# fizzy74/passport-zk-circuits

Measured on AMD Instinct MI355X. Metric: registerIdentityBuilder witnesses/sec, batch=4096, 1 & 8 MI355X; % HBM roofline, higher is better.
Workload: dtype bn254_fr (u32 limbs)

## Files before the change

### passport-zk-circuits_amd/csrc/host_api.cpp

```cpp
#include <string.h>

#include <algorithm>

#include "../../include/pzkwit.h"
#include "host_api.hpp"
#include "pos_prog.hpp"

namespace pzk {

int nsets_env(bool query) {
  const char* e = getenv("PZK_NSETS");
  const int v = e ? atoi(e) : query ? 6 : 3;
  return v < 2 ? 2 : v > PIPELINE_SETS_MAX ? PIPELINE_SETS_MAX : v;
}

bool parse_sym(const char* text, size_t len, uint64_t o0_size, std::vector<uint32_t>& inv, std::string& why) {
  std::vector<int64_t> w_of;
  size_t i = 0;
  uint64_t line = 0;
  auto num = [&](int64_t& v) -> bool {
    bool neg = false, any = false;
    v = 0;
    if (i < len && text[i] == '-') { neg = true; i++; }
    while (i < len && text[i] >= '0' && text[i] <= '9') { v = v * 10 + (text[i] - '0'); i++; any = true; if (v > (1ll << 40)) return false; }
    if (neg) v = -v;
    return any;
  };
  while (i < len) {
    line++;
    if (text[i] == '\n' || text[i] == '\r') { i++; continue; }
    int64_t sig, wit, comp;
    if (!num(sig) || i >= len || text[i++] != ',' || !num(wit) || i >= len || text[i++] != ',' || !num(comp)) {
      why = "sym line " + std::to_string(line) + ": expected signal_idx,witness_idx,component_idx,name";
      return false;
    }
    while (i < len && text[i] != '\n') i++;
    if (sig < 1 || (uint64_t)sig >= o0_size) {
      why = "sym line " + std::to_string(line) + ": signal index " + std::to_string(sig) + " outside 1.." +
            std::to_string(o0_size - 1);
      return false;
    }
    if (wit == -1) continue;
    if (wit < 1 || (uint64_t)wit >= o0_size) {
      why = "sym line " + std::to_string(line) + ": witness index " + std::to_string(wit) + " outside 1.." +
            std::to_string(o0_size - 1);
      return false;
    }
    if ((uint64_t)wit >= w_of.size()) w_of.resize(wit + 1, -1);
    if (w_of[wit] == -1 || sig < w_of[wit]) w_of[wit] = sig;
  }
  if (w_of.size() < 2) { why = "sym: no signal is kept"; return false; }
  inv.assign(w_of.size(), 0);
  for (size_t k = 1; k < w_of.size(); k++) {
    if (w_of[k] < 0) { why = "sym: witness index " + std::to_string(k) + " is not assigned"; return false; }
    inv[k] = (uint32_t)w_of[k];
  }
  return true;
}

void map_program(const Layout& lay, const std::vector<uint32_t>& inv, bool force_gather, MapProgram& out) {
  out = MapProgram();
  bool monotone = true;
  for (size_t k = 1; k < inv.size() && monotone; k++) monotone = inv[k] > inv[k - 1];
  if (!monotone || force_gather) return;
  out.direct = true;
  const size_t nw = lay.wit_size / 64 + 3;
  out.bits.assign(nw, 0);
  out.rank.assign(nw, 0);
  for (uint32_t g : inv) out.bits[g >> 6] |= 1ull << (g & 63);
  for (size_t i = 1; i < nw; i++) out.rank[i] = out.rank[i - 1] + (uint32_t)__builtin_popcountll(out.bits[i - 1]);
  auto kept = [&](uint64_t g) { return (out.bits[g >> 6] >> (g & 63)) & 1; };
  bool mix_t[POS_MAX_T + 1] = {};
  auto kept_in = [&](uint64_t a, uint64_t n) {
    uint64_t c = 0;
    for (uint64_t g = a; g < a + n; g++) c += kept(g);
    return c;
  };
  for (int e : {E_SHA, E_SHAD, E_POS, E_ECT}) {
    std::vector<Work>& wl = out.work[e];
    wl = lay.work[e];
    if (e == E_SHA || e == E_SHAD) {
      std::vector<Work> merged;
      uint64_t kept_cur = 0;
      for (const Work& wk : wl) {
        const uint64_t k = kept_in(lay.regions[wk.region].off + wk.start, wk.count);
        Work* last = merged.empty() ? nullptr : &merged.back();
        if (last && last->region == wk.region && lay.regions[wk.region].kind == RK_SHA_BLOCK &&
            last->start + last->count == wk.start && kept_cur + k <= EMIT_CHUNK) {
          last->count += wk.count;
          kept_cur += k;
        } else {
          merged.push_back(wk);
          kept_cur = k;
        }
      }
      wl.swap(merged);
    }
    for (Work& wk : wl) {
      const Region& R = lay.regions[wk.region];
      const uint32_t* src = nullptr;
      const uint16_t* src16 = nullptr;
      if (R.kind == RK_SHA_BLOCK) src = lay.sha_prog.data() + wk.start;
      else if (R.kind == RK_POSEIDON) src16 = lay.pos_prog.data() + lay.pos_prog_off[lay.pos[R.a[0]].n + 1] + wk.start;
      else if (R.kind == RK_ECT) src = lay.ec_prog.data() + lay.ec_prog_off[R.a[1]] + wk.start;
      else continue;
      wk.pad = (uint32_t)out.mprog.size();
      for (uint32_t q = 0; q < wk.count; q++)
        if (kept(R.off + wk.start + q)) {
          out.mprog.push_back(src ? src[q] : src16[q]);
          if (src16) mix_t[lay.pos[R.a[0]].n + 1] |= (pos_img_need_t(lay.pos[R.a[0]].n + 1, src16[q]) & PI_MIX) != 0;
        }
    }
  }
  for (int t = 2; t <= POS_MAX_T; t++)
    if (!mix_t[t]) out.pos_nomix |= 1u << t;
  if (out.mprog.empty()) out.mprog.push_back(0);
}

}

using namespace pzk;

extern "C" {

static int sym_check_impl(const pzk_params* params, const char* sym, size_t sym_len, uint64_t* witness_size) {
  if (!params || !sym) return api_fail(PZK_E_ARG, "null argument");
  Layout L;
  std::string why;
  if (!build_layout(*params, L, why)) return api_fail(PZK_E_PARAMS, why);
  std::vector<uint32_t> inv;
  if (!parse_sym(sym, sym_len, L.wit_size, inv, why)) return api_fail(PZK_E_ARG, why);
  if (witness_size) *witness_size = inv.size();
  return 0;
}

static int layout_query_impl(const pzk_params* params, pzk_info* info, uint32_t* n_regions) {
  if (!params || !info) return api_fail(PZK_E_ARG, "null argument");
  Layout L;
  std::string why;
  if (!build_layout(*params, L, why)) return api_fail(PZK_E_PARAMS, why);
  memset(info, 0, sizeof *info);
  info->witness_size = L.wit_size;
  info->n_inputs = L.n_inputs;
  info->n_outputs = L.n_outputs;
  info->n_public_inputs = L.n_public;
  info->n_input_groups = (uint32_t)L.inputs.size();
  info->pipeline_depth = nsets_env(params->circuit == PZK_CIRCUIT_QUERY);
  if (n_regions) *n_regions = (uint32_t)L.regions.size();
  return 0;
}

static int layout_region_impl(const pzk_params* params, uint32_t i, uint64_t* off, uint32_t* len, uint32_t* kind) {
  if (!params) return api_fail(PZK_E_ARG, "null argument");
  Layout L;
  std::string why;
  if (!build_layout(*params, L, why)) return api_fail(PZK_E_PARAMS, why);
  if (i >= L.regions.size()) return api_fail(PZK_E_ARG, "region index out of range");
  if (off) *off = L.regions[i].off;
  if (len) *len = L.regions[i].len;
  if (kind) *kind = L.regions[i].kind;
  return 0;
}

int pzk_sym_check(const pzk_params* params, const char* sym, size_t sym_len, uint64_t* witness_size) {
  return guarded([&] { return sym_check_impl(params, sym, sym_len, witness_size); });
}

int pzk_layout_query(const pzk_params* params, pzk_info* info, uint32_t* n_regions) {
  return guarded([&] { return layout_query_impl(params, info, n_regions); });
}

int pzk_layout_region(const pzk_params* params, uint32_t i, uint64_t* off, uint32_t* len, uint32_t* kind) {
  return guarded([&] { return layout_region_impl(params, i, off, len, kind); });
}

}
```

### passport-zk-circuits_amd/csrc/kernels.hip

```cpp
#include <hip/hip_runtime.h>
#include <stdlib.h>
#include <string.h>

#include "poseidon.hpp"
#include "regcore.hpp"
#include "smt_chain4.hpp"
#include "pss.hpp"
#include "regemit.hpp"
#include "sha.hpp"
#include "sha1.hpp"
#include "sha512.hpp"
#include "sha_prog.hpp"
#include "mapsink.hpp"
#include "kernels.hpp"

namespace pzk {

__global__ void k_load_values(const ValueLoad* loads, int n_loads, const uint8_t* inputs, uint64_t n_inputs,
                              fr* values, uint32_t batch) {
  uint32_t w = blockIdx.x * blockDim.x + threadIdx.x;
  int l = blockIdx.y;
  if (w >= batch || l >= n_loads) return;
  ValueLoad ld = loads[l];
  fr x = load_fr(inputs + 32ull * ((uint64_t)w * n_inputs + ld.in_off));
  values[(size_t)ld.slot * batch + w] = fr_to_mont(x);
}

__global__ void __launch_bounds__(64, 1) k_sha_core(const ShaJob* jobs, int n_jobs, const uint8_t* inputs, uint64_t n_inputs,
                           const uint8_t* derived, uint64_t n_derived, uint32_t* sha_core, uint32_t core_words,
                           int32_t* status, uint32_t batch) {
  core_priority();
  uint32_t w = blockIdx.x * blockDim.x + threadIdx.x;
  int j = blockIdx.y;
  if (w >= batch || j >= n_jobs) return;
  const ShaJob& J = jobs[j];
  const uint8_t* row = J.src ? derived + 32ull * (uint64_t)w * n_derived : inputs + 32ull * (uint64_t)w * n_inputs;
  if (J.algo == 1) sha1_core_lane(row, J, sha_core + (size_t)w * core_words, status ? status + w : nullptr);
  else if (J.algo >= 3) sha512_core_lane(row, J, sha_core + (size_t)w * core_words, status ? status + w : nullptr);
  else sha_core_lane(row, J, sha_core + (size_t)w * core_words, status ? status + w : nullptr);
}

__device__ __forceinline__ uint64_t sha_own_sig(const Region& R, const uint32_t* H , uint32_t s,
                                                bool& is_copy, uint64_t& src) {
  const int B = R.a[1];
  const uint32_t inLen = 512u * B, O = R.a[4] == 224 ? 224u : 256u;
  is_copy = false;
  if (R.a[3]) {
    if (s < O) { uint32_t j = s >> 5, i = s & 31; return (H[B * 8 + j] >> (31 - i)) & 1; }
    s -= O;
    if (s < inLen) { is_copy = true; src = (uint64_t)R.a[2] + s; return 0; }
    s -= inLen;
  }
  if (s < O) { uint32_t j = s >> 5, i = s & 31; return (H[B * 8 + j] >> (31 - i)) & 1; }
  s -= O;
  if (s < inLen) { is_copy = true; src = (uint64_t)R.a[2] + s; return 0; }
  s -= inLen;
  if (s < 256u * (B + 1)) { uint32_t m = s >> 8, j = (s >> 5) & 7, i = s & 31; return (H[m * 8 + j] >> i) & 1; }
  s -= 256u * (B + 1);
  return ((O == 224 ? SHA224_IV[s >> 5] : SHA_IV[s >> 5]) >> (s & 31)) & 1;
}

template <int SHA_U, int MM>
__global__ void __launch_bounds__(EMIT_THREADS) k_emit_sha(DevLayout L, const Work* work, const uint8_t* inputs,
                                                          const uint8_t* derived, const uint32_t* sha_core,
                                                          uint8_t* wtns, size_t stride, int wit_major) {
  __shared__ uint32_t core[SHA_BLOCK_CORE + 8 * 65];
  __shared__ __attribute__((aligned(16))) uint64_t wt[SHA_WT_SIZE];
  const Work wk = work[wit_major ? blockIdx.y : blockIdx.x];
  const uint32_t w = wit_major ? blockIdx.x : blockIdx.y;
  const Region R = L.regions[wk.region];
  const ShaJob job = L.sha[R.a[0]];
  const uint32_t* wc = sha_core + (size_t)w * L.sha_core_words + job.core_off;
  const OutRow out = out_row(L, wtns, stride, w, R.off + wk.start);
  if (R.kind == RK_SHA_BLOCK) {
    const uint32_t* bc = wc + R.a[1] * SHA_BLOCK_CORE;
    for (int i = threadIdx.x; i < SHA_BLOCK_CORE; i += blockDim.x) core[i] = bc[i];
    __syncthreads();
    const ShaBlk Bk{core};
    const uint32_t a = wk.start, b = wk.start + wk.count - 1;
    auto rng = [](uint32_t lo_sig, uint32_t per, int nr, uint32_t x) {
      return x < lo_sig ? 0 : (int)min((x - lo_sig) / per, (uint32_t)nr - 1);
    };
    const bool sch = a < SHA_SCH_ROUND0 + 48 * SHA_SCH_ROUND_SIGS && b >= SHA_SCH_ROUND0;
    const bool cmp = a < SHA_RDS_CMP0 + 64 * SHA_CMP_SIGS && b >= SHA_RDS_CMP0;
    const int r0 = sch ? rng(SHA_SCH_ROUND0, SHA_SCH_ROUND_SIGS, 48, a) : 0;
    const int r1 = sch ? rng(SHA_SCH_ROUND0, SHA_SCH_ROUND_SIGS, 48, b) + 1 : 0;
    const int k0 = cmp ? rng(SHA_RDS_CMP0, SHA_CMP_SIGS, 64, a) : 0;
    const int k1 = cmp ? rng(SHA_RDS_CMP0, SHA_CMP_SIGS, 64, b) + 1 : 0;
    const int n_base = SHA_WT_SCH, n_ff = 16, n_sch = (r1 - r0) * SHA_SCH_WORDS, n_cmp = (k1 - k0) * SHA_CMP_WORDS;
    for (int v = threadIdx.x; v < n_base + n_ff + n_sch + n_cmp; v += blockDim.x) {
      int e = v < n_base ? v
            : v < n_base + n_ff ? SHA_WT_FF32 + (v - n_base)
            : v < n_base + n_ff + n_sch ? SHA_WT_SCH + r0 * SHA_SCH_WORDS + (v - n_base - n_ff)
                                        : SHA_WT_CMP + k0 * SHA_CMP_WORDS + (v - n_base - n_ff - n_sch);
      wt[e] = sha_wt_entry(Bk, e);
    }
    __syncthreads();
    const DescRun dr = desc_run<MM>(L, wtns, stride, w, wk, R.off + wk.start, L.sha_prog + wk.start);
    const uint32_t* prog = dr.prog;
    const uint32_t tot = 2 * dr.count;
    for (uint32_t base = threadIdx.x; base < tot; base += SHA_U * blockDim.x) {
      uint32_t d[SHA_U];
#pragma unroll
      for (int k = 0; k < SHA_U; k++) {
        const uint32_t h = base + k * blockDim.x;
        d[k] = h < tot ? prog[h >> 1] : 0u;
      }
#pragma unroll
      for (int k = 0; k < SHA_U; k++) {
        const uint32_t h = base + k * blockDim.x;
        const uint64_t v = (h & 1) ? 0 : sha_desc_apply(d[k], wt[d[k] & 2047]);
        store_half<MAP_O0>(dr.out, h, make_uint4((uint32_t)v, (uint32_t)(v >> 32), 0u, 0u), h < tot);
      }
    }
  } else {
    const int Bn = R.a[1];
    for (int i = threadIdx.x; i < 8 * (Bn + 1); i += blockDim.x) {
      int m = i >> 3, j = i & 7;
      core[i] = m < Bn ? wc[m * SHA_BLOCK_CORE + j] : wc[Bn * SHA_BLOCK_CORE + j];
    }
    __syncthreads();
    const uint8_t* in_row = job.src ? derived + 32ull * (uint64_t)w * L.n_derived : inputs + 32ull * (uint64_t)w * L.n_inputs;
    uint4* stage = reinterpret_cast<uint4*>(wt);
    emit_run<MM>(out, wk.count, stage, [&](uint32_t q) {
      bool cp; uint64_t src = 0;
      uint64_t v = sha_own_sig(R, core, wk.start + q, cp, src);
      return cp ? el_load(in_row + 32ull * src) : el_u64(v);
    });
  }
}

__global__ void __launch_bounds__(EMIT_THREADS) k_emit_sha1(DevLayout L, const Work* work, const uint8_t* inputs,
                                                           const uint8_t* derived, const uint32_t* sha_core,
                                                           uint8_t* wtns, size_t stride) {
  __shared__ uint32_t wd[5 + 80 + 85];
  __shared__ uint4 stage[2 * EMIT_THREADS];
  const Work wk = work[blockIdx.y];
  const uint32_t w = blockIdx.x;
  const Region R = L.regions[wk.region];
  const ShaJob job = L.sha[R.a[0]];
  const uint32_t* wc = sha_core + (size_t)w * L.sha_core_words + job.core_off;
  const OutRow out = out_row(L, wtns, stride, w, R.off + wk.start);
  if (R.kind == RK_SHA1_BLOCK) {
    const uint32_t* bc = wc + R.a[1] * SHA1_BLOCK_CORE;
    for (int i = threadIdx.x; i < SHA1_BLOCK_CORE; i += blockDim.x) wd[i < 85 ? i : i + 5] = bc[i];
    if (threadIdx.x == 0) {
      wd[89] = bc[0]; wd[88] = bc[1];
      wd[87] = rol32(bc[2], 2); wd[86] = rol32(bc[3], 2); wd[85] = rol32(bc[4], 2);
    }
    __syncthreads();
    const Sha1Blk X{wd, wd + 5, wd + 85};
    emit_run(out, wk.count, stage, [&](uint32_t q) { return el_u64(sha1_block_sig(X, wk.start + q)); });
  } else {
    const int Bn = R.a[1];
    const uint32_t* hout = wc + Bn * SHA1_BLOCK_CORE;
    const uint8_t* in_row = job.src ? derived + 32ull * (uint64_t)w * L.n_derived : inputs + 32ull * (uint64_t)w * L.n_inputs;
    emit_run(out, wk.count, stage, [&](uint32_t q) {
      bool cp;
      const uint64_t v = sha1_own_sig(hout, Bn, R.a[3] != 0, wk.start + q, cp);
      return cp ? el_load(in_row + 32ull * (R.a[2] + v)) : el_u64(v);
    });
  }
}

__device__ __forceinline__ El el_u128v(U128 v) {
  return El{make_uint4((uint32_t)v.lo, (uint32_t)(v.lo >> 32), (uint32_t)v.hi, (uint32_t)(v.hi >> 32)), make_uint4(0u, 0u, 0u, 0u)};
}
__global__ void __launch_bounds__(EMIT_THREADS) k_emit_sha512(DevLayout L, const Work* work, const uint8_t* inputs,
                                                             const uint8_t* derived, const uint32_t* sha_core,
                                                             uint8_t* wtns, size_t stride) {
  __shared__ uint64_t wd[8 + 80 + 84 + 84];
  __shared__ uint4 stage[2 * EMIT_THREADS];
  const Work wk = work[blockIdx.y];
  const uint32_t w = blockIdx.x;
  const Region R = L.regions[wk.region];
  const ShaJob job = L.sha[R.a[0]];
  const uint64_t* wc = reinterpret_cast<const uint64_t*>(sha_core + (size_t)w * L.sha_core_words + job.core_off);
  const OutRow out = out_row(L, wtns, stride, w, R.off + wk.start);
  if (R.kind == RK_SHA5_BLOCK) {
    const uint64_t* bc = wc + (size_t)R.a[1] * (SHA5_BLOCK_CORE / 2);
    for (int i = threadIdx.x; i < 8 + 80; i += blockDim.x) wd[i] = bc[i];
    for (int i = threadIdx.x; i < 80; i += blockDim.x) { wd[88 + 4 + i] = bc[88 + i]; wd[172 + 4 + i] = bc[168 + i]; }
    if (threadIdx.x < 4) {
      wd[88 + threadIdx.x] = bc[3 - threadIdx.x];
      wd[172 + threadIdx.x] = bc[7 - threadIdx.x];
    }
    __syncthreads();
    const Sha5Blk X{wd, wd + 8, wd + 88, wd + 172};
    emit_run(out, wk.count, stage, [&](uint32_t q) { return el_u128v(sha5_block_sig(X, wk.start + q)); });
  } else {
    const int Bn = R.a[1], O = R.a[3];
    const uint8_t* in_row = job.src ? derived + 32ull * (uint64_t)w * L.n_derived : inputs + 32ull * (uint64_t)w * L.n_inputs;
    const uint64_t* iv = job.algo == 3 ? SHA384_IV_ : SHA512_IV_;
    auto hin = [&](int m, uint32_t j) -> uint64_t { return m < Bn ? wc[(size_t)m * (SHA5_BLOCK_CORE / 2) + j] : wc[(size_t)Bn * (SHA5_BLOCK_CORE / 2) + j]; };
    emit_run(out, wk.count, stage, [&](uint32_t q) {
// ... 253 lines not shown
```

### passport-zk-circuits_amd/csrc/sha_prog.hpp

```cpp
#pragma once
#include <stdint.h>

namespace pzk {

constexpr int SHA_WT_W = 0;
__host__ __device__ constexpr int sha_wt_a(int k) { return 67 + k; }
__host__ __device__ constexpr int sha_wt_e(int k) { return 135 + k; }
constexpr int SHA_WT_K = 203;
constexpr int SHA_WT_SCH = 267;
constexpr int SHA_SCH_WORDS = 11;
enum { SW_X7, SW_Y18, SW_Z3, SW_T0, SW_S0, SW_X17, SW_Y19, SW_Z10, SW_T1, SW_S1, SW_V };
constexpr int SHA_WT_CMP = SHA_WT_SCH + 48 * SHA_SCH_WORDS;
constexpr int SHA_CMP_WORDS = 15;
enum { CW_CH, CW_S1, CW_S0, CW_MJ, CW_OVE, CW_OVA, CW_R2, CW_R13, CW_R22, CW_T0, CW_R6, CW_R11, CW_R25, CW_T1, CW_XY };
constexpr int SHA_WT_FF32 = SHA_WT_CMP + 64 * SHA_CMP_WORDS;
constexpr int SHA_WT_FF64 = SHA_WT_FF32 + 8;
constexpr int SHA_WT_SIZE = SHA_WT_FF64 + 8;

constexpr uint32_t SHA_D_EXTRACT = 0, SHA_D_MASK = 1;
__host__ __device__ constexpr uint32_t sha_desc(int idx, int lo, int n, uint32_t mode) {
  return (uint32_t)idx | ((uint32_t)lo << 11) | ((uint32_t)n << 17) | (mode << 24);
}
__host__ __device__ inline uint64_t sha_desc_apply(uint32_t d, uint64_t v) {
  const uint32_t lo = (d >> 11) & 63, n = (d >> 17) & 127;
  const uint64_t m = n >= 64 ? ~0ull : ((1ull << n) - 1);
  return (d >> 24) ? (v & (m << lo)) : ((v >> lo) & m);
}

constexpr uint32_t SHA_BLOCK_SIGNALS_COUNT = 36048 + 114714;
constexpr uint32_t SHA_SCH_ROUND0 = 3648, SHA_SCH_ROUND_SIGS = 675;
constexpr uint32_t SHA_RDS_CMP0 = 36048 + 13258 + 704, SHA_CMP_SIGS = 1548;

}
```

### passport-zk-circuits_amd/csrc/fr.hpp

```cpp
#pragma once
#include <hip/hip_runtime.h>
#include <stdint.h>

namespace pzk {

struct fr { uint32_t v[8]; };

constexpr uint32_t P_[8] = {0xf0000001u, 0x43e1f593u, 0x79b97091u, 0x2833e848u,
                                                 0x8181585du, 0xb85045b6u, 0xe131a029u, 0x30644e72u};
constexpr uint32_t R2_[8] = {0xae216da7u, 0x1bb8e645u, 0xe35c59e3u, 0x53fe3ab1u,
                                                  0x53bb8085u, 0x8c49833du, 0x7f4e44a5u, 0x0216d0b1u};
constexpr uint32_t R1_[8] = {0x4ffffffbu, 0xac96341cu, 0x9f60cd29u, 0x36fc7695u,
                                                  0x7879462eu, 0x666ea36fu, 0x9a07df2fu, 0x0e0a77c1u};
constexpr uint32_t PINV = 0xefffffffu;

__device__ __forceinline__ fr fr_zero() { fr r; for (int i = 0; i < 8; i++) r.v[i] = 0; return r; }
__device__ __forceinline__ fr fr_u64(uint64_t x) {
  fr r = fr_zero(); r.v[0] = (uint32_t)x; r.v[1] = (uint32_t)(x >> 32); return r;
}
__device__ __forceinline__ fr fr_const(const uint32_t (&c)[8]) { fr r; for (int i = 0; i < 8; i++) r.v[i] = c[i]; return r; }
__device__ __forceinline__ fr fr_mont_one() { return fr_const(R1_); }

__device__ __forceinline__ uint32_t fr_bit(const fr& a, int i) {
  uint32_t r = 0;
// ... 242 lines not shown
__device__ __forceinline__ fr fr_shfl(const fr& a, int src, int width) {
  fr r;
#pragma unroll
  for (int k = 0; k < 8; k++) r.v[k] = (uint32_t)__shfl((int)a.v[k], src, width);
  return r;
}
__device__ __forceinline__ fr fr_shfl_up(const fr& a, unsigned d) {
  fr r;
#pragma unroll
  for (int k = 0; k < 8; k++) r.v[k] = (uint32_t)__shfl_up((int)a.v[k], d, 64);
  return r;
}
__device__ __forceinline__ fr fr_shfl_down(const fr& a, unsigned d) {
  fr r;
#pragma unroll
  for (int k = 0; k < 8; k++) r.v[k] = (uint32_t)__shfl_down((int)a.v[k], d, 64);
  return r;
}

template <int G>
__device__ __forceinline__ void fr_group_others(const fr& acc, fr& others, fr& total) {
  static_assert(G >= 2 && G <= 64 && (G & (G - 1)) == 0, "G: a power of two <= 64");
  const int l = (int)(threadIdx.x & (G - 1));
  auto up = [](const fr& a, int d) { fr r; for (int k = 0; k < 8; k++) r.v[k] = (uint32_t)__shfl_up((int)a.v[k], d, G); return r; };
  auto down = [](const fr& a, int d) { fr r; for (int k = 0; k < 8; k++) r.v[k] = (uint32_t)__shfl_down((int)a.v[k], d, G); return r; };
  fr p = acc, s = acc;
#pragma unroll
  for (int d = 1; d < G; d <<= 1) {
    const fr u = up(p, d), v = down(s, d);
    if (l >= d) p = fr_mul(p, u);
    if (l + d < G) s = fr_mul(s, v);
  }
  fr pe = up(p, 1), se = down(s, 1);
  if (l == 0) pe = fr_mont_one();
  if (l == G - 1) se = fr_mont_one();
  others = fr_mul(pe, se);
  total = fr_shfl(p, G - 1, G);
}

struct El { uint4 lo, hi; };
__device__ __forceinline__ El el_zero() { return El{make_uint4(0u, 0u, 0u, 0u), make_uint4(0u, 0u, 0u, 0u)}; }
__device__ __forceinline__ El el_u64(uint64_t v) {
  return El{make_uint4((uint32_t)v, (uint32_t)(v >> 32), 0u, 0u), make_uint4(0u, 0u, 0u, 0u)};
}
__device__ __forceinline__ El el_fr(const fr& a) {
  return El{make_uint4(a.v[0], a.v[1], a.v[2], a.v[3]), make_uint4(a.v[4], a.v[5], a.v[6], a.v[7])};
}
__device__ __forceinline__ El el_load(const uint8_t* src) {
  const uint4* s = reinterpret_cast<const uint4*>(src);
  return El{s[0], s[1]};
}
__device__ __forceinline__ void wave_sync() {
  __builtin_amdgcn_fence(__ATOMIC_RELEASE, "wavefront");
  __builtin_amdgcn_wave_barrier();
  __builtin_amdgcn_fence(__ATOMIC_ACQUIRE, "wavefront");
}
template <int SW = 128>
__device__ __forceinline__ void wave_store(uint8_t* wave_out, const El& e, uint32_t nvalid, uint4* stage) {
  const uint32_t lane = threadIdx.x & 63;
  uint4* d = reinterpret_cast<uint4*>(wave_out);
  if constexpr (SW == 128) {
    stage[2 * lane] = e.lo;
    stage[2 * lane + 1] = e.hi;
    wave_sync();
    const uint4 a = stage[lane], b = stage[64 + lane];
    if (lane < 2 * nvalid) d[lane] = a;
    if (64 + lane < 2 * nvalid) d[64 + lane] = b;
    wave_sync();
  } else {
    static_assert(SW == 64, "stage: 128 or 64 uint4 per wave");
#pragma unroll
    for (uint32_t h = 0; h < 2; h++) {
      if ((lane >> 5) == h) {
        stage[2 * (lane & 31)] = e.lo;
        stage[2 * (lane & 31) + 1] = e.hi;
      }
      wave_sync();
      const uint4 a = stage[lane];
      if (64 * h + lane < 2 * nvalid) d[64 * h + lane] = a;
      wave_sync();
    }
  }
}
template <int SW = 128, typename F>
__device__ __forceinline__ void emit_run(uint8_t* out, uint32_t count, uint4* stage_block, F f) {
  const uint32_t lane = threadIdx.x & 63;
  uint4* stage = stage_block + (threadIdx.x >> 6) * SW;
  for (uint32_t q0 = threadIdx.x - lane; q0 < count; q0 += blockDim.x) {
    const uint32_t q = q0 + lane;
    const El e = q < count ? f(q) : el_zero();
    wave_store<SW>(out + 32ull * q0, e, count - q0 < 64 ? count - q0 : 64, stage);
  }
}

__device__ __forceinline__ void store_u64(uint8_t* dst, uint64_t v) {
  uint4* d = reinterpret_cast<uint4*>(dst);
  d[0] = make_uint4((uint32_t)v, (uint32_t)(v >> 32), 0u, 0u);
  d[1] = make_uint4(0u, 0u, 0u, 0u);
}
__device__ __forceinline__ void store_fr(uint8_t* dst, const fr& a) {
  uint4* d = reinterpret_cast<uint4*>(dst);
  d[0] = make_uint4(a.v[0], a.v[1], a.v[2], a.v[3]);
  d[1] = make_uint4(a.v[4], a.v[5], a.v[6], a.v[7]);
}
__device__ __forceinline__ fr load_fr(const uint8_t* src) {
  const uint4* s = reinterpret_cast<const uint4*>(src);
  uint4 a = s[0], b = s[1];
  fr r; r.v[0] = a.x; r.v[1] = a.y; r.v[2] = a.z; r.v[3] = a.w; r.v[4] = b.x; r.v[5] = b.y; r.v[6] = b.z; r.v[7] = b.w;
  return r;
}

__device__ __forceinline__ void core_priority() { __builtin_amdgcn_s_setprio(3); }

__device__ __forceinline__ void lane_status(int32_t* st, int32_t code) {
  if (!st) return;
  int32_t old = *(volatile int32_t*)st;
  while (old == 0 || old > code) {
    int32_t seen = atomicCAS(st, old, code);
    if (seen == old) return;
    old = seen;
  }
}

}
```

### passport-zk-circuits_amd/csrc/mapsink.hpp

```cpp
#pragma once
#include "fr.hpp"
#include "layout.hpp"

namespace pzk {

typedef __attribute__((address_space(4))) const uint64_t cu64_t;
typedef __attribute__((address_space(4))) const uint32_t cu32_t;

struct MapWin {
  uint64_t w0, w1;
  uint32_t r0, r1;
  uint64_t base;
};
__device__ __forceinline__ MapWin map_win(const KeepMap& M, uint64_t g0) {
  const uint32_t i = __builtin_amdgcn_readfirstlane((uint32_t)(g0 >> 6));
  cu64_t* b = (cu64_t*)M.bits;
  cu32_t* r = (cu32_t*)M.rank;
  MapWin m;
  m.w0 = b[i];
  m.w1 = b[i + 1];
  m.r0 = r[i];
  m.r1 = r[i + 1];
  m.base = (uint64_t)i << 6;
  return m;
}
__device__ __forceinline__ bool map_keep(const MapWin& m, uint64_t g) {
  const uint32_t d = (uint32_t)(g - m.base);
  return ((d < 64 ? m.w0 : m.w1) >> (d & 63)) & 1;
}
__device__ __forceinline__ uint32_t map_rank(const MapWin& m, uint64_t g) {
  const uint32_t d = (uint32_t)(g - m.base);
  const uint64_t w = d < 64 ? m.w0 : m.w1;
  return (d < 64 ? m.r0 : m.r1) + (uint32_t)__popcll(w & ((1ull << (d & 63)) - 1));
}
__device__ __forceinline__ bool map_keep_lane(const KeepMap& M, uint64_t g, uint32_t& rank) {
  const uint64_t w = M.bits[g >> 6];
  rank = M.rank[g >> 6] + (uint32_t)__popcll(w & ((1ull << (g & 63)) - 1));
  return (w >> (g & 63)) & 1;
}

enum { MAP_O0 = 0, MAP_DIRECT = 1, MAP_ANY = 2 };

struct OutRow {
  uint8_t* row;
  uint64_t g;
  KeepMap map;
  __device__ OutRow at(uint64_t q) const { return OutRow{row, g + q, map}; }
};
__device__ __forceinline__ OutRow out_row(const DevLayout& L, uint8_t* wtns, size_t stride, uint32_t w, uint64_t g) {
  return OutRow{wtns + (size_t)w * stride, g, L.keep};
}

template <int MM = MAP_ANY>
__device__ __forceinline__ void store_half(const OutRow& o, uint32_t h, const uint4& v, bool valid) {
  if (MM == MAP_O0 || (MM == MAP_ANY && !o.map.bits)) {
    if (valid) reinterpret_cast<uint4*>(o.row + 32ull * o.g)[h] = v;
    return;
  }
  const uint32_t lane = threadIdx.x & 63;
  const MapWin m = map_win(o.map, o.g + ((h - lane) >> 1));
  const uint64_t e = o.g + (h >> 1);
  if (valid && map_keep(m, e)) reinterpret_cast<uint4*>(o.row)[2ull * map_rank(m, e) + (h & 1)] = v;
}

__device__ __forceinline__ uint32_t map_rank_at(const KeepMap& M, uint64_t g) {
  const uint32_t i = __builtin_amdgcn_readfirstlane((uint32_t)(g >> 6));
  const uint64_t w = ((cu64_t*)M.bits)[i];
  return ((cu32_t*)M.rank)[i] + (uint32_t)__popcll(w & ((1ull << (g & 63)) - 1));
}

template <typename T, typename P>
__device__ __forceinline__ uint32_t kept_collect(const OutRow& o, uint32_t a, uint32_t n, T* list, P payload) {
  const uint64_t lo = o.g + a, hi = lo + n;
  const uint32_t r0 = map_rank_at(o.map, lo), nk = map_rank_at(o.map, hi) - r0;
  const uint32_t lane = threadIdx.x & 63, nw = blockDim.x >> 6;
  const uint32_t i0 = (uint32_t)(lo >> 6), i1 = (uint32_t)((hi - 1) >> 6);
  for (uint32_t i = i0 + __builtin_amdgcn_readfirstlane(threadIdx.x >> 6); i <= i1; i += nw) {
    const uint32_t iu = __builtin_amdgcn_readfirstlane(i);
    const uint64_t word = ((cu64_t*)o.map.bits)[iu];
    const uint32_t rk = ((cu32_t*)o.map.rank)[iu];
    const uint64_t e = ((uint64_t)iu << 6) + lane;
    if (((word >> lane) & 1) && e >= lo && e < hi)
      list[rk + (uint32_t)__popcll(word & ((1ull << lane) - 1)) - r0] = payload((uint32_t)(e - lo));
  }
  __syncthreads();
  return nk;
}

constexpr uint32_t MAP_SEG = 1664;
template <uint32_t SEG = MAP_SEG>
__device__ __forceinline__ uint16_t* map_seg_list() {
  __shared__ uint16_t klist[SEG];
  return klist;
}

template <int MM = MAP_ANY, bool LANE_INDEP = true, int SW = 128, uint32_t SEG = MAP_SEG, typename F>
__device__ __forceinline__ void emit_run(const OutRow& o, uint32_t count, uint4* stage_block, F f) {
  if (MM == MAP_O0 || (MM == MAP_ANY && !o.map.bits)) {
    emit_run<SW>(o.row + 32ull * o.g, count, stage_block, f);
    return;
  }
  const uint32_t lane = threadIdx.x & 63;
  uint4* stage = stage_block + (threadIdx.x >> 6) * SW;
  if constexpr (LANE_INDEP) {
    uint16_t* klist = map_seg_list<SEG>();
    for (uint32_t a = 0; a < count; a += SEG) {
      const uint32_t n = min(SEG, count - a);
      const uint32_t r0 = map_rank_at(o.map, o.g + a);
      const uint32_t nk = kept_collect(o, a, n, klist, [](uint32_t q) { return (uint16_t)q; });
      uint8_t* dst = o.row + 32ull * r0;
      for (uint32_t k0 = threadIdx.x - lane; k0 < nk; k0 += blockDim.x) {
        const uint32_t k = k0 + lane;
        const El e = k < nk ? f(a + klist[k]) : el_zero();
        wave_store<SW>(dst + 32ull * k0, e, nk - k0 < 64 ? nk - k0 : 64, stage);
      }
      __syncthreads();
    }
  } else {
    for (uint32_t q0 = threadIdx.x - lane; q0 < count; q0 += blockDim.x) {
      const uint32_t q = q0 + lane;
      const MapWin m = map_win(o.map, o.g + q0);
      const bool keep = q < count && map_keep(m, o.g + q);
      const uint64_t mask = __ballot(keep);
      if (mask == 0) continue;
      const El e = q < count ? f(q) : el_zero();
      const uint32_t pos = (uint32_t)__popcll(mask & ((1ull << lane) - 1)), nk = (uint32_t)__popcll(mask);
      uint4* d = reinterpret_cast<uint4*>(o.row + 32ull * map_rank(m, o.g + q0));
      if constexpr (SW == 128) {
        if (keep) {
          stage[2 * pos] = e.lo;
          stage[2 * pos + 1] = e.hi;
        }
        wave_sync();
        const uint4 a = stage[lane], b = stage[64 + lane];
        if (lane < 2 * nk) d[lane] = a;
        if (64 + lane < 2 * nk) d[64 + lane] = b;
        wave_sync();
      } else {
#pragma unroll
        for (uint32_t h = 0; h < 2; h++) {
          if (keep && (pos >> 5) == h) {
            stage[2 * (pos & 31)] = e.lo;
            stage[2 * (pos & 31) + 1] = e.hi;
          }
          wave_sync();
          const uint4 a = stage[lane];
          if (64 * h + lane < 2 * nk) d[64 * h + lane] = a;
          wave_sync();
        }
      }
    }
  }
}

struct DescRun {
  const uint32_t* prog;
  uint32_t count;
  OutRow out;
};
template <int MM>
__device__ __forceinline__ DescRun desc_run(const DevLayout& L, uint8_t* wtns, size_t stride, uint32_t w, const Work& wk,
                                            uint64_t g, const uint32_t* o0_prog) {
  uint8_t* row = wtns + (size_t)w * stride;
  if (MM == MAP_O0 || (MM == MAP_ANY && !L.keep.bits)) return DescRun{o0_prog, wk.count, OutRow{row, g, KeepMap{nullptr, nullptr}}};
  const uint32_t r0 = map_rank_at(L.keep, g), r1 = map_rank_at(L.keep, g + wk.count);
  return DescRun{L.mprog + wk.pad, r1 - r0, OutRow{row, r0, KeepMap{nullptr, nullptr}}};
}

}
```

### passport-zk-circuits_amd/csrc/regemit.hpp

```cpp
#pragma once
#include "bufs.hpp"
#include "fr.hpp"
#include "layout.hpp"
#include "poseidon.hpp"
#include "regcore.hpp"
#include "sha.hpp"
#include "mm_prog.hpp"
#include "ec_emit.hpp"
#include "pss.hpp"
#include "mapsink.hpp"
#include "query.hpp"

namespace pzk {


struct W256 { uint32_t v[8]; };
__device__ __forceinline__ W256 w_zero() { W256 r; for (int i = 0; i < 8; i++) r.v[i] = 0; return r; }
__device__ __forceinline__ W256 w_u64(uint64_t x) { W256 r = w_zero(); r.v[0] = (uint32_t)x; r.v[1] = (uint32_t)(x >> 32); return r; }
__device__ __forceinline__ W256 w_mask(const W256& a, int nbits) {
  W256 r = a;
#pragma unroll
  for (int i = 0; i < 8; i++) {
    int lo = 32 * i;
    if (nbits <= lo) r.v[i] = 0;
// ... 597 lines not shown
      hi += C.kt_hi[tb + j] + (lo < v ? 1u : 0u);
    }
  };
  if (p >= 2u * N) {
    const int k = (int)p - 2 * N;
    if (lvl == 0) return el_u64(k < N ? C.x[k] : C.y[k - N]);
    uint64_t lo, hi;
    val(k >= N ? 1 : 0, k >= N ? k - N : k, lo, hi);
    return el_u128(lo, hi);
  }
  if (p == 2u * N - 1) return el_zero();
  if (lvl == 0) return el_w(u192w(u192_at(C.cxy, (int)p)));
  if (lvl <= K64_OL) return el_w(u192w(ko5_at(ko, kt_base64(lvl) + m * 2 * N + (int)p)));
  const int lo_u = (int)p < N ? 0 : (int)p - N + 1, hi_u = (int)p < N ? (int)p : N - 1;
  U192 acc;
  for (int u = lo_u; u <= hi_u; u++) {
    uint64_t al, ah, bl, bh;
    val(0, u, al, ah);
    val(1, (int)p - u, bl, bh);
    mac2(acc, al, ah, bl, bh);
  }
  return el_w(u192w(acc));
}

template <int K, int SEC>
__device__ __forceinline__ El mm_el(const MMCore& C, uint32_t s) {
  if constexpr (SEC == MM_MODCHK) {
    const uint32_t i = s / 129, t = s - 129 * i;
    return el_num2bits(C.r[i], 0, 64, t);
  } else if constexpr (SEC == MM_LT) {
    const uint32_t i = s / 140;
    uint32_t t = s - 140 * i;
    const uint64_t a = C.n[i], b = C.r[i];
    if (t < 134) {
      const uint64_t vlo = a - b, vhi = a >= b ? 1u : 0u;
      if (t < 3) return el_u64(t == 0 ? 1 - vhi : t == 1 ? a : b);
      return el_num2bits(vlo, vhi, 65, t - 3);
    }
    t -= 134;
    if (t == 0 || t == 3) return el_u64(a == b);
    if (t == 1) return el_u64(a);
    if (t == 2) return el_u64(b);
    if (t == 4) return a <= b ? el_u64(b - a) : el_fr(fr_sub(fr_zero(), fr_u64(a - b)));
    const uint64_t* iv = C.inv + 4 * i;
    return El{make_uint4((uint32_t)iv[0], (uint32_t)(iv[0] >> 32), (uint32_t)iv[1], (uint32_t)(iv[1] >> 32)),
              make_uint4((uint32_t)iv[2], (uint32_t)(iv[2] >> 32), (uint32_t)iv[3], (uint32_t)(iv[3] >> 32))};
  } else if constexpr (SEC == MM_RANGE) {
    constexpr uint32_t RL = 128 + mm_log_ceil(2 * K) + 3 - 64, PER = 2 * RL + 1;
    const uint32_t i = s / PER, t = s - PER * i;
    const uint64_t lo = C.cr[2 * i], hi = C.cr[2 * i + 1] + (1ull << (RL - 1 - 64));
    return el_num2bits(lo, hi, RL, t);
  } else if constexpr (SEC == MM_KARA && K == KT_K) {
    return kara_el32(C, C.ko, s);
  } else if constexpr (SEC == MM_KARA && K == 64) {
    return kara_el64(C, C.ko, s);
  } else if constexpr (SEC == MM_KARA) {
    static_assert((K & (K - 1)) != 0, "KaratsubaOverflow sizes have their own table path");
    return el_w(mm_sig(C, ((uint32_t)SEC << 24) | s));
  } else if constexpr (SEC == MM_Q) {
    return el_u64(C.q[s]);
  } else if constexpr (SEC == MM_R) {
    return el_u64(C.r[s]);
  } else if constexpr (SEC == MM_TMPM) {
    const uint32_t i = s / K, j = s - i * K;
    U192 acc;
    acc.mac(C.q[i], C.n[j]);
    return el_w(u192w(acc));
  } else {
    return el_w(mm_sig(C, ((uint32_t)SEC << 24) | s));
  }
}

#ifdef PZK_MM_PROF
static __device__ unsigned long long g_mm_prof[MM_SECTIONS + 2];
#define PZK_MM_CLK(v) const long long v = clock64()
#define PZK_MM_ACC(i, t0) do { const long long t1_ = clock64(); if (threadIdx.x == 0) atomicAdd(&g_mm_prof[i], (unsigned long long)(t1_ - (t0))); } while (0)
#else
#define PZK_MM_CLK(v)
#define PZK_MM_ACC(i, t0)
#endif

constexpr int MM_STAGE = 64;
constexpr uint32_t MM_SEG = 896;
template <int K, int SEC, int MM>
__device__ __forceinline__ void mm_sections(const MMCore C, const OutRow& out, uint4* stage) {
  if constexpr (SEC < (int)MM_SECTIONS) {
    constexpr MMStarts S = mm_starts(K);
    constexpr uint32_t a = S.v[SEC], n = S.v[SEC + 1] - S.v[SEC];
    PZK_MM_CLK(t0);
    constexpr bool INDEP = !(SEC == MM_TMPR || (SEC == MM_KARA && (K & (K - 1)) != 0));
    emit_run<MM, INDEP, MM_STAGE, MM_SEG>(out.at(a), n, stage, [=](uint32_t q) { return mm_el<K, SEC>(C, q); });
    PZK_MM_ACC(SEC, t0);
    mm_sections<K, SEC + 1, MM>(C, out, stage);
  }
}

template <int K, int MM, int NT = 256>
__global__ void __launch_bounds__(NT) k_emit_mm(DevLayout L, const Work* work, Bufs B) {
  __shared__ uint64_t lds[MM_CORE_WORDS(K) + K + 3 * (4 * K - 1)];
  PZK_MM_CLK(tp);
  const Work wk = work[blockIdx.x];
  const uint32_t w = blockIdx.y;
  const Region R = L.regions[wk.region];
  const uint64_t* mc = B.rsa_core + (size_t)w * L.rsa_core_words + (size_t)R.a[0] * MM_CORE_WORDS(K);
  const uint8_t* row = B.inputs + 32ull * (uint64_t)w * L.n_inputs;
#ifdef PZK_MM_SERIAL_LOAD
  for (int i = threadIdx.x; i < MM_CORE_WORDS(K); i += blockDim.x) lds[i] = mc[i];
  for (int i = threadIdx.x; i < K; i += blockDim.x) lds[MM_CORE_WORDS(K) + i] = in_u64(row + 32ull * (R.a[1] + i));
#else
  constexpr int MM_NT = NT, CW = MM_CORE_WORDS(K), CL = (CW + MM_NT - 1) / MM_NT;
  uint64_t cv[CL];
#pragma unroll
  for (int k = 0; k < CL; k++) {
    const int i = threadIdx.x + k * MM_NT;
    cv[k] = mc[i < CW ? i : 0];
  }
  const uint64_t xin = in_u64(row + 32ull * (R.a[1] + (threadIdx.x < K ? threadIdx.x : 0)));
#pragma unroll
  for (int k = 0; k < CL; k++) {
    const int i = threadIdx.x + k * MM_NT;
    if (i < CW) lds[i] = cv[k];
  }
  if (threadIdx.x < K) lds[CW + threadIdx.x] = xin;
#endif
  __syncthreads();
  uint64_t* cxy = lds + MM_CORE_WORDS(K) + K;
  uint64_t* cqn = cxy + 3 * (2 * K - 1);
  for (int c = threadIdx.x; c < 4 * K - 1; c += blockDim.x) {
    U192 acc;
    if (c < 2 * K - 1) {
      for (int j = c < K ? 0 : c - K + 1; j <= c && j < K; j++) acc.mac(lds[j], lds[K + (c - j)]);
      cxy[3 * c] = acc.a0; cxy[3 * c + 1] = acc.a1; cxy[3 * c + 2] = acc.a2;
    } else {
      const int i = c - (2 * K - 1);
      for (int j = i < K ? 0 : i - K + 1; j <= i && j <= K; j++) acc.mac(lds[2 * K + j], lds[MM_CORE_WORDS(K) + (i - j)]);
      cqn[3 * i] = acc.a0; cqn[3 * i + 1] = acc.a1; cqn[3 * i + 2] = acc.a2;
    }
  }
  __syncthreads();
  constexpr int KTN = K == KT_K ? KT_VALUES : K == 64 ? K64_TL_VALUES : 1;
  __shared__ uint64_t kt_lo[KTN];
  __shared__ uint8_t kt_hi[KTN];
  if (K == KT_K || K == 64) {
    int base = 0, pbase = 0, nodes = 3;
    for (int l = 1; l <= (K == KT_K ? KT_LEVELS : K64_TL); l++) {
      const int N = K >> l, cnt = nodes * 2 * N;
      for (int r = threadIdx.x; r < cnt; r += blockDim.x) {
        const int m = r / (2 * N), k = r - m * 2 * N, op = k >= N, u = k - op * N, p = m / 3, c = m - 3 * p;
        uint64_t alo, ahi, blo = 0, bhi = 0;
        if (l == 1) {
          const uint64_t* src = op ? lds + K : lds;
          alo = src[u]; ahi = 0; if (c != 0) { blo = src[u + N]; bhi = 0; }
        } else {
          const int pi = pbase + p * 4 * N + op * 2 * N + u;
          alo = kt_lo[pi]; ahi = kt_hi[pi];
          if (c != 0) { blo = kt_lo[pi + N]; bhi = kt_hi[pi + N]; }
        }
        uint64_t lo, hi;
        if (c == 0) { lo = alo; hi = ahi; }
        else if (c == 1) { lo = blo; hi = bhi; }
        else { lo = alo + blo; hi = ahi + bhi + (lo < alo); }
        kt_lo[base + r] = lo; kt_hi[base + r] = (uint8_t)hi;
      }
      __syncthreads();
      pbase = base;
      base += cnt;
      nodes *= 3;
    }
  }
  constexpr int KON = K == KT_K ? 3 * KO_VALUES : K == 64 ? 3 * K64_OL_VALUES : 1;
  __shared__ uint32_t ko[(KON + 2) / 3 * 5];
  if (K == KT_K || K == 64) {
    for (int r = threadIdx.x; r < (K == KT_K ? KO_VALUES : K64_OL_VALUES); r += blockDim.x) {
      const int l = K == KT_K ? (r < 96 ? 1 : r < 240 ? 2 : 3) : (r < kt_base64(2) ? 1 : 2), N = K >> l;
      const int lb = K == KT_K ? kt_level_base(l) : kt_base64(l), rr = r - lb, m = rr / (2 * N);
      const int p = rr - m * 2 * N, tb = lb + m * 2 * N;
      U192 acc;
      if (p < 2 * N - 1)
        for (int u = p < N ? 0 : p - N + 1; u <= (p < N ? p : N - 1); u++)
          mac2(acc, kt_lo[tb + u], kt_hi[tb + u], kt_lo[tb + N + p - u], kt_hi[tb + N + p - u]);
      uint32_t* o = ko + 5 * r;
      o[0] = (uint32_t)acc.a0; o[1] = (uint32_t)(acc.a0 >> 32); o[2] = (uint32_t)acc.a1; o[3] = (uint32_t)(acc.a1 >> 32);
      o[4] = (uint32_t)acc.a2;
    }
    __syncthreads();
  }
  MMCore C{K, lds, lds + K, lds + 2 * K, lds + 3 * K + 1, lds + MM_CORE_WORDS(K), lds + 4 * K + 1, lds + 8 * K + 1,
           cxy, cqn, (K & (K - 1)) == 0, K == KT_K || K == 64 ? kt_lo : nullptr, K == KT_K || K == 64 ? kt_hi : nullptr,
           K == KT_K || K == 64 ? ko : nullptr};
  const OutRow out = out_row(L, B.wtns, B.stride, w, R.off + wk.start);
  __shared__ uint4 stage[MM_STAGE * (NT / 64)];
  PZK_MM_ACC(MM_SECTIONS, tp);
  mm_sections<K, 0, MM>(C, out, stage);
}

enum BjjRec { BR_X1, BR_Y1, BR_OX, BR_OY, BR_INV, BR_X1Y2, BR_Y1X2, BR_DELTA, BR_TAU, BR_XYD, BR_DELTAD, BR_TAUD,
              BR_NX1, BR_NY1, BR_N };
enum BjjConst { BC_ZERO, BC_ONE, BC_B8X, BC_B8Y, BC_INVB8X, BC_N };

__device__ __forceinline__ uint32_t bjj_step_of(uint32_t s) { return s < 46 ? 0 : 1 + (s - 46) / 60; }
__device__ __forceinline__ uint32_t bjj_sig_of(uint32_t i) { return i == 0 ? 0 : 46 + 60 * (i - 1); }

#ifndef PZK_TEMPLATE_KERNELS_ONLY
__global__ void __launch_bounds__(256, 6) k_emit_bjj(DevLayout L, const Work* work, Bufs B) {
  constexpr int CB = (BJJ_EMIT_STEPS + 1) * BR_N;
  __shared__ fr rec[CB + BC_N];
  __shared__ uint32_t bits[BJJ_EMIT_STEPS + 1], zx1[BJJ_EMIT_STEPS + 1];
  const Work wk = work[blockIdx.x];
  const uint32_t w = blockIdx.y;
  const Region R = L.regions[wk.region];
  const fr* core = B.bjj_core + (size_t)w * L.bjj_core_fr;
  const uint32_t i0 = bjj_step_of(wk.start), i1 = bjj_step_of(wk.start + wk.count - 1) + 1;
  const int base = i0 == 0 ? 0 : (int)i0 - 1;
  const int nrec = (int)i1 - base;
  {
    fr skm = B.vs.at(L.reg.v_sk, w);
    fr sk = fr_from_mont_fast(skm);
    for (int j = threadIdx.x; j < nrec; j += blockDim.x) {
      int i = base + j;
      bits[j] = fr_bit(sk, 253 - i);
    }
    if (threadIdx.x < BC_N) {
      const int c = (int)threadIdx.x;
      rec[CB + c] = c == BC_ZERO ? fr_zero() : c == BC_ONE ? fr_u64(1) : c == BC_B8X ? fr_const(BJJ_B8X)
                  : c == BC_B8Y ? fr_const(BJJ_B8Y) : fr_const(BJJ_INV_B8X);
    }
  }
  __syncthreads();
  for (int q = threadIdx.x; q < nrec * BR_N; q += blockDim.x) {
    const int v = q / nrec, j = q - v * nrec, i = base + j;
    const fr* P = core + 5 * i;
    fr r;
    if (v == BR_XYD || v == BR_DELTAD || v == BR_TAUD) {
      if (i == 0) r = fr_zero();
      else {
        fr xp = P[-3], yp = P[-2];
        fr xy = fr_mul_fast(xp, yp);
        if (v == BR_XYD) r = xy;
        else if (v == BR_DELTAD) r = fr_mul_fast(fr_sub(yp, fr_mul_fast(fr_to_mont(fr_u64(BJJ_A)), xp)), fr_add(xp, yp));
        else r = fr_sqr_fast(xy);
      }
    } else if (v == BR_OX || v == BR_OY) {
      r = P[v];
    } else {
      const bool bit = bits[j];
      fr x1 = i == 0 ? fr_zero() : P[0], y1 = i == 0 ? fr_zero() : P[1];
      fr x2 = bit ? fr_to_mont(fr_const(BJJ_B8X)) : fr_zero(), y2 = bit ? fr_to_mont(fr_const(BJJ_B8Y)) : fr_zero();
      switch (v) {
        case BR_X1: r = x1; zx1[j] = fr_is_zero(x1); break;
        case BR_Y1: r = y1; break;
        case BR_NX1: r = fr_sub(fr_zero(), x1); break;
        case BR_NY1: r = fr_sub(fr_zero(), y1); break;
        case BR_INV: r = i == 0 ? fr_zero() : P[4]; break;
        case BR_X1Y2: r = fr_mul_fast(x1, y2); break;
        case BR_Y1X2: r = fr_mul_fast(y1, x2); break;
        case BR_DELTA: r = fr_mul_fast(fr_sub(y1, fr_mul_fast(fr_to_mont(fr_u64(BJJ_A)), x1)), fr_add(x2, y2)); break;
        default: r = fr_mul_fast(fr_mul_fast(x1, y2), fr_mul_fast(y1, x2)); break;
      }
    }
    rec[j * BR_N + v] = fr_from_mont_fast(r);
  }
  __syncthreads();
  const OutRow out = out_row(L, B.wtns, B.stride, w, R.off + wk.start);
  __shared__ uint4 stage[2 * 256];
  emit_run(out, wk.count, stage, [&](uint32_t q) -> El {
    const uint32_t s = wk.start + q, i = bjj_step_of(s), t = s - bjj_sig_of(i);
    const int j = (int)i - base;
    const int rc = j * BR_N, rp = rc - BR_N;
    constexpr int ZERO = CB + BC_ZERO, ONE = CB + BC_ONE;
    int idx;
    if (t >= 46) {
      const uint32_t u = t - 46;
      idx = u < 2 ? rc + BR_X1 + (int)u : u < 4 ? rp + BR_OX + (int)u - 2 : u < 6 ? rc + BR_X1 + (int)u - 4
          : u < 10 ? rp + BR_OX + (int)(u & 1) : u < 12 ? rc + BR_XYD : rc + (u == 12 ? BR_DELTAD : BR_TAUD);
    } else {
      const bool bit = bits[j] != 0, z1 = zx1[j] != 0, z2 = !bit;
// ... 33 lines not shown
```

Before: 82340.

## Precompute branchless SHA descriptors and use buffer stores in the mapped emit loop

```diff
diff --git a/passport-zk-circuits_amd/csrc/host_api.cpp b/passport-zk-circuits_amd/csrc/host_api.cpp
--- a/passport-zk-circuits_amd/csrc/host_api.cpp
+++ b/passport-zk-circuits_amd/csrc/host_api.cpp
@@ -5,6 +5,7 @@
 #include "../../include/pzkwit.h"
 #include "host_api.hpp"
 #include "pos_prog.hpp"
+#include "sha_prog.hpp"
 
 namespace pzk {
 
@@ -107,7 +108,7 @@
       wk.pad = (uint32_t)out.mprog.size();
       for (uint32_t q = 0; q < wk.count; q++)
         if (kept(R.off + wk.start + q)) {
-          out.mprog.push_back(src ? src[q] : src16[q]);
+          out.mprog.push_back(R.kind == RK_SHA_BLOCK ? sha_mdesc_of(src[q]) : src ? src[q] : src16[q]);
           if (src16) mix_t[lay.pos[R.a[0]].n + 1] |= (pos_img_need_t(lay.pos[R.a[0]].n + 1, src16[q]) & PI_MIX) != 0;
         }
     }
diff --git a/passport-zk-circuits_amd/csrc/kernels.hip b/passport-zk-circuits_amd/csrc/kernels.hip
--- a/passport-zk-circuits_amd/csrc/kernels.hip
+++ b/passport-zk-circuits_amd/csrc/kernels.hip
@@ -97,20 +97,64 @@
     }
     __syncthreads();
     const DescRun dr = desc_run<MM>(L, wtns, stride, w, wk, R.off + wk.start, L.sha_prog + wk.start);
-    const uint32_t* prog = dr.prog;
-    const uint32_t tot = 2 * dr.count;
-    for (uint32_t base = threadIdx.x; base < tot; base += SHA_U * blockDim.x) {
-      uint32_t d[SHA_U];
+    if constexpr (MM == MAP_O0) {
+      const uint32_t* prog = dr.prog;
+      const uint32_t tot = 2 * dr.count;
+      for (uint32_t base = threadIdx.x; base < tot; base += SHA_U * blockDim.x) {
+        uint32_t d[SHA_U];
 #pragma unroll
-      for (int k = 0; k < SHA_U; k++) {
-        const uint32_t h = base + k * blockDim.x;
-        d[k] = h < tot ? prog[h >> 1] : 0u;
+        for (int k = 0; k < SHA_U; k++) {
+          const uint32_t h = base + k * blockDim.x;
+          d[k] = h < tot ? prog[h >> 1] : 0u;
+        }
+#pragma unroll
+        for (int k = 0; k < SHA_U; k++) {
+          const uint32_t h = base + k * blockDim.x;
+          const uint64_t v = (h & 1) ? 0 : sha_desc_apply(d[k], wt[d[k] & 2047]);
+          store_half<MAP_O0>(dr.out, h, make_uint4((uint32_t)v, (uint32_t)(v >> 32), 0u, 0u), h < tot);
+        }
       }
-#pragma unroll
-      for (int k = 0; k < SHA_U; k++) {
-        const uint32_t h = base + k * blockDim.x;
-        const uint64_t v = (h & 1) ? 0 : sha_desc_apply(d[k], wt[d[k] & 2047]);
-        store_half<MAP_O0>(dr.out, h, make_uint4((uint32_t)v, (uint32_t)(v >> 32), 0u, 0u), h < tot);
+    } else {
+      constexpr uint32_t T = EMIT_THREADS, BATCH = SHA_U * T;
+      constexpr int SHA_G = 4;
+      typedef uint32_t u32x4 __attribute__((ext_vector_type(4)));
+      const uint32_t tot = 2 * dr.count, n_full = tot / BATCH;
+      const char* prog = reinterpret_cast<const char*>(dr.prog);
+      const __amdgpu_buffer_rsrc_t rs = __builtin_amdgcn_make_buffer_rsrc(dr.out.row + 32ull * dr.out.g, 0, 16 * tot, 0x20000);
+      uint32_t s_off = 0;
+      const uint32_t p_off = 4u * (threadIdx.x >> 1), d_off = 16u * threadIdx.x;
+      const uint64_t ones = (threadIdx.x & 1) ? 0ull : ~0ull;
+      uint32_t zero = 0;
+      asm volatile("" : "+v"(zero));
+      const char* wtb = reinterpret_cast<const char*>(wt);
+      auto desc = [&](int k) { return *reinterpret_cast<const uint32_t*>((prog + 2u * T * k) + p_off); };
+      auto word = [&](uint32_t d) { return *reinterpret_cast<const uint64_t*>(wtb + sha_mdesc_wt_byte(d)); };
+      auto put = [&](int k, uint32_t d, uint64_t wv) {
+        const uint64_t v = sha_mdesc_apply(d, wv, ones);
+        __builtin_amdgcn_raw_buffer_store_b128(u32x4{(uint32_t)v, (uint32_t)(v >> 32), zero, zero}, rs, d_off + (s_off + 16u * T * k), 0, 0);
+      };
+      for (uint32_t b = 0; b < n_full; b++, prog += 2 * BATCH, s_off += 16 * BATCH) {
+        uint32_t d[SHA_U];
+  #pragma unroll
+        for (int k = 0; k < SHA_U; k++) d[k] = desc(k);
+  #pragma unroll
+        for (int g = 0; g < SHA_U; g += SHA_G) {
+          uint64_t wv[SHA_G];
+  #pragma unroll
+          for (int k = 0; k < SHA_G; k++) wv[k] = word(d[g + k]);
+  #pragma unroll
+          for (int k = 0; k < SHA_G; k++) put(g + k, d[g + k], wv[k]);
+          __builtin_amdgcn_sched_barrier(0);
+        }
+      }
+      {
+        const uint32_t left = tot - n_full * BATCH;
+        uint32_t d[SHA_U];
+  #pragma unroll
+        for (int k = 0; k < SHA_U; k++) d[k] = threadIdx.x + k * T < left ? desc(k) : 0u;
+  #pragma unroll
+        for (int k = 0; k < SHA_U; k++)
+          if (threadIdx.x + k * T < left) put(k, d[k], word(d[k]));
       }
     }
   } else {
diff --git a/passport-zk-circuits_amd/csrc/sha_prog.hpp b/passport-zk-circuits_amd/csrc/sha_prog.hpp
--- a/passport-zk-circuits_amd/csrc/sha_prog.hpp
+++ b/passport-zk-circuits_amd/csrc/sha_prog.hpp
@@ -27,6 +27,22 @@
   return (d >> 24) ? (v & (m << lo)) : ((v >> lo) & m);
 }
 
+__host__ __device__ constexpr uint32_t sha_mdesc(int idx, int lo, int n, uint32_t mode) {
+  return (uint32_t)lo | ((uint32_t)(64 - n) << 6) | ((mode == SHA_D_MASK ? (uint32_t)lo : 0u) << 12) | ((uint32_t)idx << 21);
+}
+__host__ __device__ constexpr uint32_t sha_mdesc_of(uint32_t d) {
+  return sha_mdesc((int)(d & 2047), (int)((d >> 11) & 63),
+                   ((d >> 17) & 127) >= 64 || ((d >> 17) & 127) == 0 ? 64 : (int)((d >> 17) & 127), d >> 24);
+}
+__host__ __device__ constexpr uint32_t sha_mdesc_idx(uint32_t d) { return d >> 21; }
+__host__ __device__ constexpr uint32_t sha_mdesc_wt_byte(uint32_t d) { return d >> 18; }
+__host__ __device__ constexpr uint32_t sha_mdesc_lo(uint32_t d) { return d & 63; }
+__host__ __device__ constexpr uint32_t sha_mdesc_n(uint32_t d) { return 64 - ((d >> 6) & 63); }
+__host__ __device__ constexpr uint32_t sha_mdesc_back(uint32_t d) { return (d >> 12) & 63; }
+__host__ __device__ inline uint64_t sha_mdesc_apply(uint32_t d, uint64_t v, uint64_t ones = ~0ull) {
+  return ((v >> (d & 63)) & (ones >> ((d >> 6) & 63))) << ((d >> 12) & 63);
+}
+
 constexpr uint32_t SHA_BLOCK_SIGNALS_COUNT = 36048 + 114714;
 constexpr uint32_t SHA_SCH_ROUND0 = 3648, SHA_SCH_ROUND_SIGS = 675;
 constexpr uint32_t SHA_RDS_CMP0 = 36048 + 13258 + 704, SHA_CMP_SIGS = 1548;
```

Measured after the change: 82290. Within noise of the previous version (-0.1%).

## Store MM witness sections via wave shuffles and rotate wave start per section

Applied to the files above, without the earlier changes.

```diff
diff --git a/passport-zk-circuits_amd/csrc/fr.hpp b/passport-zk-circuits_amd/csrc/fr.hpp
--- a/passport-zk-circuits_amd/csrc/fr.hpp
+++ b/passport-zk-circuits_amd/csrc/fr.hpp
@@ -348,14 +348,48 @@
     }
   }
 }
+__device__ __forceinline__ uint32_t run_q0(uint32_t rot) {
+  if (rot == 0) return threadIdx.x - (threadIdx.x & 63);
+  const uint32_t nw = blockDim.x >> 6, wv = __builtin_amdgcn_readfirstlane(threadIdx.x >> 6);
+  return 64 * (wv >= rot ? wv - rot : wv + nw - rot);
+}
 template <int SW = 128, typename F>
-__device__ __forceinline__ void emit_run(uint8_t* out, uint32_t count, uint4* stage_block, F f) {
+__device__ __forceinline__ void emit_run(uint8_t* out, uint32_t count, uint4* stage_block, F f, uint32_t rot = 0) {
   const uint32_t lane = threadIdx.x & 63;
   uint4* stage = stage_block + (threadIdx.x >> 6) * SW;
-  for (uint32_t q0 = threadIdx.x - lane; q0 < count; q0 += blockDim.x) {
+  for (uint32_t q0 = run_q0(rot); q0 < count; q0 += blockDim.x) {
     const uint32_t q = q0 + lane;
     const El e = q < count ? f(q) : el_zero();
     wave_store<SW>(out + 32ull * q0, e, count - q0 < 64 ? count - q0 : 64, stage);
+  }
+}
+
+__device__ __forceinline__ uint4 shfl_u4(const uint4& a, int src) {
+  return make_uint4((uint32_t)__shfl((int)a.x, src, 64), (uint32_t)__shfl((int)a.y, src, 64),
+                    (uint32_t)__shfl((int)a.z, src, 64), (uint32_t)__shfl((int)a.w, src, 64));
+}
+template <typename F>
+__device__ __forceinline__ void emit_run_shfl(uint8_t* out, uint32_t count, F f, uint32_t rot = 0) {
+  const uint32_t lane = threadIdx.x & 63;
+  const bool odd = lane & 1;
+  for (uint32_t q0 = run_q0(rot); q0 < count; q0 += blockDim.x) {
+    const uint32_t q = q0 + lane;
+    const El e = q < count ? f(q) : el_zero();
+    const uint32_t nh = 2 * (count - q0 < 64 ? count - q0 : 64);
+    const bool any_hi = __any((e.hi.x | e.hi.y | e.hi.z | e.hi.w) != 0);
+    uint4* d = reinterpret_cast<uint4*>(out + 32ull * q0);
+#pragma unroll
+    for (uint32_t r = 0; r < 2; r++) {
+      const int src = (int)(32 * r + (lane >> 1));
+      uint4 v = shfl_u4(e.lo, src);
+      if (any_hi) {
+        const uint4 w = shfl_u4(e.hi, src);
+        if (odd) v = w;
+      } else if (odd) {
+        v = make_uint4(0u, 0u, 0u, 0u);
+      }
+      if (64 * r + lane < nh) d[64 * r + lane] = v;
+    }
   }
 }
 
diff --git a/passport-zk-circuits_amd/csrc/mapsink.hpp b/passport-zk-circuits_amd/csrc/mapsink.hpp
--- a/passport-zk-circuits_amd/csrc/mapsink.hpp
+++ b/passport-zk-circuits_amd/csrc/mapsink.hpp
@@ -95,9 +95,9 @@
 }
 
 template <int MM = MAP_ANY, bool LANE_INDEP = true, int SW = 128, uint32_t SEG = MAP_SEG, typename F>
-__device__ __forceinline__ void emit_run(const OutRow& o, uint32_t count, uint4* stage_block, F f) {
+__device__ __forceinline__ void emit_run(const OutRow& o, uint32_t count, uint4* stage_block, F f, uint32_t rot = 0) {
   if (MM == MAP_O0 || (MM == MAP_ANY && !o.map.bits)) {
-    emit_run<SW>(o.row + 32ull * o.g, count, stage_block, f);
+    emit_run<SW>(o.row + 32ull * o.g, count, stage_block, f, rot);
     return;
   }
   const uint32_t lane = threadIdx.x & 63;
@@ -153,6 +153,11 @@
   }
 }
 
+template <typename F>
+__device__ __forceinline__ void emit_run_shfl(const OutRow& o, uint32_t count, F f, uint32_t rot = 0) {
+  emit_run_shfl(o.row + 32ull * o.g, count, f, rot);
+}
+
 struct DescRun {
   const uint32_t* prog;
   uint32_t count;
diff --git a/passport-zk-circuits_amd/csrc/regemit.hpp b/passport-zk-circuits_amd/csrc/regemit.hpp
--- a/passport-zk-circuits_amd/csrc/regemit.hpp
+++ b/passport-zk-circuits_amd/csrc/regemit.hpp
@@ -703,16 +703,30 @@
 
 constexpr int MM_STAGE = 64;
 constexpr uint32_t MM_SEG = 896;
-template <int K, int SEC, int MM>
+__host__ __device__ constexpr bool mm_store_shfl(int sec) {
+  return sec == MM_Q || sec == MM_R || sec == MM_XYN || sec == MM_MCOPY || sec == MM_MODCHK || sec == MM_GT0 ||
+         sec == MM_GTIN || sec == MM_LE0 || sec == MM_LEIN || sec == MM_LERES || sec == MM_M2IN || sec == MM_TMPM ||
+         sec == MM_RANGE;
+}
+__host__ __device__ constexpr uint32_t mm_section_rot(int K, int sec, uint32_t NW) {
+  uint32_t chunks = 0;
+  for (int i = 0; i < sec; i++) chunks += (mm_section_size(K, i) + 63) / 64;
+  return chunks % NW;
+}
+template <int K, int SEC, int MM, int NT>
 __device__ __forceinline__ void mm_sections(const MMCore C, const OutRow& out, uint4* stage) {
   if constexpr (SEC < (int)MM_SECTIONS) {
     constexpr MMStarts S = mm_starts(K);
     constexpr uint32_t a = S.v[SEC], n = S.v[SEC + 1] - S.v[SEC];
     PZK_MM_CLK(t0);
     constexpr bool INDEP = !(SEC == MM_TMPR || (SEC == MM_KARA && (K & (K - 1)) != 0));
-    emit_run<MM, INDEP, MM_STAGE, MM_SEG>(out.at(a), n, stage, [=](uint32_t q) { return mm_el<K, SEC>(C, q); });
+    constexpr uint32_t ROT = MM == MAP_O0 ? mm_section_rot(K, SEC, NT / 64) : 0;
+    if constexpr (MM == MAP_O0 && INDEP && mm_store_shfl(SEC))
+      emit_run_shfl(out.at(a), n, [=](uint32_t q) { return mm_el<K, SEC>(C, q); }, ROT);
+    else
+      emit_run<MM, INDEP, MM_STAGE, MM_SEG>(out.at(a), n, stage, [=](uint32_t q) { return mm_el<K, SEC>(C, q); }, ROT);
     PZK_MM_ACC(SEC, t0);
-    mm_sections<K, SEC + 1, MM>(C, out, stage);
+    mm_sections<K, SEC + 1, MM, NT>(C, out, stage);
   }
 }
 
@@ -812,7 +826,7 @@
   const OutRow out = out_row(L, B.wtns, B.stride, w, R.off + wk.start);
   __shared__ uint4 stage[MM_STAGE * (NT / 64)];
   PZK_MM_ACC(MM_SECTIONS, tp);
-  mm_sections<K, 0, MM>(C, out, stage);
+  mm_sections<K, 0, MM, NT>(C, out, stage);
 }
 
 enum BjjRec { BR_X1, BR_Y1, BR_OX, BR_OY, BR_INV, BR_X1Y2, BR_Y1X2, BR_DELTA, BR_TAU, BR_XYD, BR_DELTAD, BR_TAUD,
```

Result: slower. 81910 before, 80560 after (-1.6%).
